# pdh930105/ARCQuant

Hardware: AMD Instinct MI355X
Metric: ARC-NVFP4 GEMM TFLOP/s (M=4096, N=KQ=4096, KE=64) (higher is better)
Workload: dtype f16

## Files before the change

arcquant_amd/csrc/gemm_common.hpp:

```cpp
#pragma once
#include <hip/hip_runtime.h>
#include <stdint.h>

#include "arcq_device.hpp"

#ifdef ARCQ_PLAIN_WEIGHT_LOADS
#define ARCQ_WLOAD(ptr) (*(ptr))
#else
#define ARCQ_WLOAD(ptr) __builtin_nontemporal_load(ptr)
#endif

namespace arcq {

typedef _Float16 f16x2 __attribute__((ext_vector_type(2)));
typedef _Float16 f16x8 __attribute__((ext_vector_type(8)));
typedef float f32x4 __attribute__((ext_vector_type(4)));
typedef float f32x16 __attribute__((ext_vector_type(16)));

union Frag8 {
  f16x8 v;
  f16x2 p[4];
  uint4 u;
};

__device__ __forceinline__ f16x2 sf_pair(uint32_t byte) {
  const uint32_t h = (byte & 0x7fu) << 7;
  const uint32_t w = h | (h << 16);
  f16x2 r;
  __builtin_memcpy(&r, &w, 4);
  return r;
}

__device__ __forceinline__ f16x2 sf_pair_at(uint32_t word, uint32_t off) {
  const uint32_t w = __builtin_amdgcn_ubfe(word, off, 7u) * 0x00800080u;
  f16x2 r;
  __builtin_memcpy(&r, &w, 4);
  return r;
}

__device__ __forceinline__ Frag8 dequant8(uint32_t codes, f16x2 s2) {
  Frag8 f;
#ifdef ARCQ_EXPERIMENT_NO_SCALE_MUL
  f.p[0] = __builtin_amdgcn_cvt_scalef32_pk_f16_fp4(codes, 256.0f, 0);
  f.p[1] = __builtin_amdgcn_cvt_scalef32_pk_f16_fp4(codes, 256.0f, 1);
  f.p[2] = __builtin_amdgcn_cvt_scalef32_pk_f16_fp4(codes, 256.0f, 2);
  f.p[3] = __builtin_amdgcn_cvt_scalef32_pk_f16_fp4(codes, 256.0f, 3);
  (void)s2;
  return f;
#endif
  f.p[0] = __builtin_amdgcn_cvt_scalef32_pk_f16_fp4(codes, 256.0f, 0) * s2;
  f.p[1] = __builtin_amdgcn_cvt_scalef32_pk_f16_fp4(codes, 256.0f, 1) * s2;
  f.p[2] = __builtin_amdgcn_cvt_scalef32_pk_f16_fp4(codes, 256.0f, 2) * s2;
  f.p[3] = __builtin_amdgcn_cvt_scalef32_pk_f16_fp4(codes, 256.0f, 3) * s2;
  return f;
}

__device__ __forceinline__ int64_t sf_atom_offset(int r, int atom, int atoms_k) {
  return ((int64_t)(r >> 7) * atoms_k + atom) * 512 + (r & 31) * 16 + ((r >> 5) & 3) * 4;
}

__device__ __forceinline__ uint32_t pack_bf16x2(float a, float b) { return f32_to_bf16_bits(a) | (f32_to_bf16_bits(b) << 16); }

template <typename Idx, typename P>
__device__ __forceinline__ void store_out4(const P& p, int m, int n, const float (&d)[4]) {
  if (p.out_dtype == ARCQ_OUT_F32) {
    float* o = reinterpret_cast<float*>(p.D) + ((Idx)m * (Idx)p.N + (Idx)n);
    if (n + 3 < p.N && (p.N & 3) == 0) {
      *reinterpret_cast<float4*>(o) = make_float4(d[0], d[1], d[2], d[3]);
    } else {
      for (int r = 0; r < 4; ++r) if (n + r < p.N) o[r] = d[r];
    }
  } else {
    uint16_t* o = reinterpret_cast<uint16_t*>(p.D) + ((Idx)m * (Idx)p.N + (Idx)n);
    if (n + 3 < p.N && (p.N & 3) == 0) {
      *reinterpret_cast<uint2*>(o) = make_uint2(pack_bf16x2(d[0], d[1]), pack_bf16x2(d[2], d[3]));
    } else {
      for (int r = 0; r < 4; ++r) if (n + r < p.N) o[r] = (uint16_t)f32_to_bf16_bits(d[r]);
    }
  }
}

template <typename Idx, typename P>
__device__ __forceinline__ void finish4_pre(const P& p, float alpha, int m, int n, const float (&acc)[4], uint2 bias_bits, uint2 res_bits) {
  const uint32_t bw[2] = {bias_bits.x, bias_bits.y}, rw[2] = {res_bits.x, res_bits.y};
  float d[4];
#pragma unroll
  for (int r = 0; r < 4; ++r) {
    d[r] = alpha * acc[r];
    if (p.bias) {
      const float b = bf16_bits_to_f32((bw[r >> 1] >> (16 * (r & 1))) & 0xffffu);
      d[r] = (p.out_dtype == ARCQ_OUT_F32 ? d[r] : bf16_bits_to_f32(f32_to_bf16_bits(d[r]))) + b;
    }
    if (p.residual) {
      const float res = bf16_bits_to_f32((rw[r >> 1] >> (16 * (r & 1))) & 0xffffu);
      d[r] = (p.out_dtype == ARCQ_OUT_F32 ? d[r] : bf16_bits_to_f32(f32_to_bf16_bits(d[r]))) + res;
    }
  }
  store_out4<Idx>(p, m, n, d);
}

template <typename Idx, typename P>
__device__ __forceinline__ void finish4(const P& p, float alpha, int m, int n, const float (&acc)[4]) {
  if ((p.N & 3) == 0 && (p.bias || p.residual) && ((reinterpret_cast<uintptr_t>(p.bias) | reinterpret_cast<uintptr_t>(p.residual)) & 7) == 0) {
    uint2 b2 = make_uint2(0, 0), r2 = make_uint2(0, 0);
    if (p.bias) b2 = *reinterpret_cast<const uint2*>(p.bias + n);
    if (p.residual) r2 = *reinterpret_cast<const uint2*>(p.residual + ((Idx)m * (Idx)p.N + (Idx)n));
    finish4_pre<Idx>(p, alpha, m, n, acc, b2, r2);
    return;
  }
  float d[4];
#pragma unroll
  for (int r = 0; r < 4; ++r) {
    d[r] = alpha * acc[r];
    if (p.bias && n + r < p.N) {
      const float b = bf16_bits_to_f32(p.bias[n + r]);
      d[r] = (p.out_dtype == ARCQ_OUT_F32 ? d[r] : bf16_bits_to_f32(f32_to_bf16_bits(d[r]))) + b;
    }
    if (p.residual && n + r < p.N) {
      const float res = bf16_bits_to_f32(p.residual[(Idx)m * (Idx)p.N + (Idx)(n + r)]);
      d[r] = (p.out_dtype == ARCQ_OUT_F32 ? d[r] : bf16_bits_to_f32(f32_to_bf16_bits(d[r]))) + res;
    }
  }
  store_out4<Idx>(p, m, n, d);
}

}
```

arcquant_amd/csrc/gemm_rowblock.hip:

```cpp
#include <hip/hip_runtime.h>
#include <stdint.h>
#include <stdlib.h>

#include "arcq_internal.hpp"
#include "gemm_common.hpp"
#include "rowblock_split.hpp"

namespace arcq {

struct RowblockParams {
  const uint8_t* A;
  const uint8_t* SFA;
  const uint8_t* RW;
  const uint8_t* RSF;
  void* D;
  const float* alpha_dev;
  const uint16_t* bias;
  const uint16_t* residual;
  int M, N, K;
  float alpha_host;
  int out_dtype;
  int pairs;
  int row_blocks;
  int slices;
  int a_stride;
  unsigned int* silu_slots;
};

typedef uint32_t rb_u32x4 __attribute__((ext_vector_type(4)));
struct RowblockRegs {
  rb_u32x4 b0, b1;
  uint32_t s;
};

constexpr int kRbWaves = 8, kRbThreads = kRbWaves * 64;

template <int kUnits, bool kSiluAbsmax>
__global__ __launch_bounds__(kRbThreads, 4) void gemm_rowblock_kernel(RowblockParams p) {
  extern __shared__ __attribute__((aligned(16))) unsigned char smem[];
  unsigned char* const a_img = smem;
  float* const red = reinterpret_cast<float*>(smem);

  const int tid = threadIdx.x, lane = tid & 63, wave = tid >> 6;
  const int q = lane >> 4, rl = lane & 15;
  const int bpw = kRbWaves / p.slices;
  const int rb = blockIdx.x * bpw + wave / p.slices;
  const int slice = wave % p.slices;
  const bool active = rb < p.row_blocks;
  int pr_begin, pr_count;
  rowblock_slice_range(p.pairs, p.slices, slice, &pr_begin, &pr_count);
  const int npairs = active ? pr_count : 0;
  const float alpha = p.alpha_host * (p.alpha_dev ? *p.alpha_dev : 1.0f);

  const int upr = p.pairs * 8, real = p.K >> 5;
  const int atoms_k = p.K >> 6;
  const int units = p.M * upr;
  uint4 qv_pre[kUnits];
  uint32_t sf_pre[kUnits];
#pragma unroll
  for (int j = 0; j < kUnits; ++j) {
    const int u = min(tid + j * kRbThreads, units - 1);
    const int m = u / upr, c = min(u - m * upr, real - 1);
    qv_pre[j] = *reinterpret_cast<const uint4*>(p.A + (size_t)m * (p.K >> 1) + c * 16);
    sf_pre[j] = *reinterpret_cast<const uint32_t*>(p.SFA + sf_atom_offset(m, c >> 1, atoms_k));
  }

  const int rbc = active ? rb : 0;
  const int pr_load = rowblock_load_base(pr_begin, npairs);
  const uint8_t* wp = p.RW + ((size_t)rbc * p.pairs + pr_load) * 2048 + lane * 16;
  const uint8_t* sp = p.RSF + ((size_t)rbc * p.pairs + pr_load) * 256 + lane * 4;
  const int last = npairs > 0 ? npairs - 1 : 0;
  int issued = 0;
  auto issue = [&](RowblockRegs& r) __attribute__((always_inline)) {
    const int i = min(issued, last);
    r.b0 = ARCQ_WLOAD(reinterpret_cast<const rb_u32x4*>(wp + (size_t)i * 2048));
    r.b1 = ARCQ_WLOAD(reinterpret_cast<const rb_u32x4*>(wp + (size_t)i * 2048 + 1024));
    r.s = ARCQ_WLOAD(reinterpret_cast<const uint32_t*>(sp + (size_t)i * 256));
    ++issued;
  };
  RowblockRegs r0, r1, r2;
  issue(r0);
  issue(r1);
  issue(r2);

  auto put_unit = [&](int u, uint4 qv, uint32_t sf) __attribute__((always_inline)) {
    const int m = u / upr, c = u - m * upr;
    uint4 f0 = make_uint4(0, 0, 0, 0), f1 = f0, f2 = f0, f3 = f0;
    if (c < real) {
      sf >>= (c & 1) * 16;
      const f16x2 s0 = sf_pair_at(sf, 0), s1 = sf_pair_at(sf, 8);
      f0 = dequant8(qv.x, s0).u; f1 = dequant8(qv.y, s0).u; f2 = dequant8(qv.z, s1).u; f3 = dequant8(qv.w, s1).u;
    }
    uint4* dst = reinterpret_cast<uint4*>(a_img + (size_t)m * p.a_stride + c * 64);
    dst[0] = f0; dst[1] = f1; dst[2] = f2; dst[3] = f3;
  };
#pragma unroll
  for (int j = 0; j < kUnits; ++j) {
    const int u = tid + j * kRbThreads;
    if (u < units) put_unit(u, qv_pre[j], sf_pre[j]);
  }
  for (int u = tid + kUnits * kRbThreads; u < units; u += kRbThreads) {
    const int m = u / upr, c = min(u - m * upr, real - 1);
    put_unit(u, *reinterpret_cast<const uint4*>(p.A + (size_t)m * (p.K >> 1) + c * 16),
             *reinterpret_cast<const uint32_t*>(p.SFA + sf_atom_offset(m, c >> 1, atoms_k)));
  }
  __syncthreads();

  f32x4 acc = {0.f, 0.f, 0.f, 0.f};
  const unsigned char* a_lane = a_img + (size_t)min(rl, p.M - 1) * p.a_stride + (size_t)pr_begin * 512 + q * 64;
  int done = 0;
  auto tile = [&](rb_u32x4 b, uint32_t s16, const unsigned char* ap) __attribute__((always_inline)) {
    Frag8 a0, a1, a2, a3;
    a0.u = *reinterpret_cast<const uint4*>(ap);
    a1.u = *reinterpret_cast<const uint4*>(ap + 16);
    a2.u = *reinterpret_cast<const uint4*>(ap + 32);
    a3.u = *reinterpret_cast<const uint4*>(ap + 48);
    const f16x2 s0 = sf_pair_at(s16, 0), s1 = sf_pair_at(s16, 8);
    const Frag8 b0 = dequant8(b.x, s0), b1 = dequant8(b.y, s0), b2 = dequant8(b.z, s1), b3 = dequant8(b.w, s1);
    acc = __builtin_amdgcn_mfma_f32_16x16x32_f16(b0.v, a0.v, acc, 0, 0, 0);
    acc = __builtin_amdgcn_mfma_f32_16x16x32_f16(b1.v, a1.v, acc, 0, 0, 0);
    acc = __builtin_amdgcn_mfma_f32_16x16x32_f16(b2.v, a2.v, acc, 0, 0, 0);
    acc = __builtin_amdgcn_mfma_f32_16x16x32_f16(b3.v, a3.v, acc, 0, 0, 0);
  };
  auto step = [&](RowblockRegs& r) __attribute__((always_inline)) {
    const unsigned char* ap = a_lane + (size_t)done * 512;
    tile(r.b0, r.s, ap);
    tile(r.b1, r.s >> 16, ap + 256);
    issue(r);
    __builtin_amdgcn_sched_barrier(0);
    ++done;
  };
  typedef uint32_t rb_u32x2 __attribute__((ext_vector_type(2)));
  rb_u32x2 ep_bias = {0, 0}, ep_res = {0, 0};
  const bool ep_pre = !kSiluAbsmax && (p.N & 3) == 0 && (p.bias || p.residual);
  if (ep_pre && slice == 0 && active && rl < p.M && rb * 16 + 4 * q < p.N) {
    const int n0p = rb * 16 + 4 * q;
    if (p.bias) ep_bias = *reinterpret_cast<const rb_u32x2*>(p.bias + n0p);
    if (p.residual) ep_res = *reinterpret_cast<const rb_u32x2*>(p.residual + (size_t)rl * p.N + n0p);
  }
#pragma unroll 1
  while (done + 3 <= npairs) {
    step(r0);
    step(r1);
    step(r2);
  }
  if (done < npairs) step(r0);
  if (done < npairs) step(r1);

  float sum[4] = {acc[0], acc[1], acc[2], acc[3]};
  if (p.slices > 1) {
    __syncthreads();
    *reinterpret_cast<float4*>(red + (wave * 64 + lane) * 4) = make_float4(sum[0], sum[1], sum[2], sum[3]);
    __syncthreads();
    if (slice != 0) return;
    for (int s2 = 1; s2 < p.slices; ++s2) {
      const float4 v = *reinterpret_cast<const float4*>(red + ((wave + s2) * 64 + lane) * 4);
      sum[0] += v.x; sum[1] += v.y; sum[2] += v.z; sum[3] += v.w;
    }
  }
  const int n0 = rb * 16 + 4 * q;
  if (active && rl < p.M && n0 < p.N) {
    if (ep_pre) finish4_pre<uint32_t>(p, alpha, rl, n0, sum, make_uint2(ep_bias.x, ep_bias.y), make_uint2(ep_res.x, ep_res.y));
    else finish4<uint32_t>(p, alpha, rl, n0, sum);
  }
  if constexpr (kSiluAbsmax) {
    uint32_t m = 0;
    if (active && rl < p.M && n0 < p.N) {
      const uint32_t b0 = f32_to_bf16_bits(alpha * sum[0]), b1 = f32_to_bf16_bits(alpha * sum[1]);
      const uint32_t b2 = f32_to_bf16_bits(alpha * sum[2]), b3 = f32_to_bf16_bits(alpha * sum[3]);
      m = max(silu_mul_bf16(b0, b1) & 0x7fffu, silu_mul_bf16(b2, b3) & 0x7fffu);
    }
#pragma unroll
    for (int sh = 32; sh > 0; sh >>= 1) m = max(m, (uint32_t)__shfl_down((int)m, sh, 64));
    if (lane == 0 && active) p.silu_slots[rb] = m;
  }
}

struct RowblockActRegs {
  rb_u32x4 a0, a1;
  uint32_t s0, s1;
};

template <bool kSiluAbsmax>
__global__ __launch_bounds__(kRbThreads, 2) void gemm_rowblock_direct_kernel(RowblockParams p) {
  extern __shared__ __attribute__((aligned(16))) unsigned char smem[];
  float* const red = reinterpret_cast<float*>(smem);

  const int tid = threadIdx.x, lane = tid & 63, wave = tid >> 6;
  const int q = lane >> 4, rl = lane & 15;
  const int bpw = kRbWaves / p.slices;
  const int rb = blockIdx.x * bpw + wave / p.slices;
  const int slice = wave % p.slices;
  const bool active = rb < p.row_blocks;
  int pr_begin, pr_count;
  rowblock_slice_range(p.pairs, p.slices, slice, &pr_begin, &pr_count);
  const int npairs = active ? pr_count : 0;
  const float alpha = p.alpha_host * (p.alpha_dev ? *p.alpha_dev : 1.0f);

  const int rbc = active ? rb : 0;
  const int pr_load = rowblock_load_base(pr_begin, npairs);
  const uint8_t* wp = p.RW + ((size_t)rbc * p.pairs + pr_load) * 2048 + lane * 16;
  const uint8_t* sp = p.RSF + ((size_t)rbc * p.pairs + pr_load) * 256 + lane * 4;
  const int tok = min(rl, p.M - 1);
  const int atoms_k = p.K >> 6, tiles_k = p.K >> 7;
  const uint8_t* arow = p.A + (size_t)tok * (p.K >> 1) + q * 16;
  const uint8_t* srow = p.SFA + sf_atom_offset(tok, 0, atoms_k) + (q & 1) * 2;
  const int last = npairs > 0 ? npairs - 1 : 0;
  int issued = 0;
  auto issue = [&](RowblockRegs& r, RowblockActRegs& x) __attribute__((always_inline)) {
    const int i = min(issued, last);
    const int t0 = 2 * (pr_load + i), t1 = t0 + 1;
    const int halfk = (p.K & 64) ? 1 : 0;
    auto a_off = [&](int t) __attribute__((always_inline)) -> size_t {
      const int tc = min(t, tiles_k - 1 + halfk);
      size_t off = (size_t)tc * 64;
      if (halfk && tc == tiles_k && q >= 2) off -= 32;
      return off;
    };
    auto s_off = [&](int t) __attribute__((always_inline)) -> size_t {
      const int atom = min(2 * t + (q >> 1), atoms_k - 1);
      return (size_t)atom * 512;
    };
    x.a0 = *reinterpret_cast<const rb_u32x4*>(arow + a_off(t0));
    x.a1 = *reinterpret_cast<const rb_u32x4*>(arow + a_off(t1));
    x.s0 = *reinterpret_cast<const uint16_t*>(srow + s_off(t0));
    x.s1 = *reinterpret_cast<const uint16_t*>(srow + s_off(t1));
    r.b0 = ARCQ_WLOAD(reinterpret_cast<const rb_u32x4*>(wp + (size_t)i * 2048));
    r.b1 = ARCQ_WLOAD(reinterpret_cast<const rb_u32x4*>(wp + (size_t)i * 2048 + 1024));
    r.s = ARCQ_WLOAD(reinterpret_cast<const uint32_t*>(sp + (size_t)i * 256));
    ++issued;
// ... 156 lines not shown
```

arcquant_amd/csrc/gemm_stream.hip:

```cpp
#include <type_traits>
#include <hip/hip_runtime.h>
#include <stdint.h>
#include <stdlib.h>

#include "arcq_internal.hpp"
#include "gemm_common.hpp"
#include "quantize_device.hpp"
#include "stream_split.hpp"

namespace arcq {

#ifdef ARCQ_STREAM_STAMPS
static unsigned long long* g_stream_stamps = nullptr;
extern "C" void arcq_debug_set_stream_stamps(void* p) { g_stream_stamps = reinterpret_cast<unsigned long long*>(p); }
#define ARCQ_STAMP(i)                                                                                                   \
  do {                                                                                                                  \
    if (p.stamps) {                                                                                                     \
      __builtin_amdgcn_sched_barrier(0);                                                                                \
      unsigned long long t_;                                                                                            \
      asm volatile("s_memtime %0\n\ts_waitcnt lgkmcnt(0)" : "=s"(t_)::"memory");                                        \
      __builtin_amdgcn_sched_barrier(0);                                                                                \
      if (lane == 0) p.stamps[((size_t)blockIdx.x * kStreamWaves + wave) * 16 + (i)] = t_;                               \
    }                                                                                                                   \
  } while (0)
#define ARCQ_STAMP_RT(i)                                                                                                \
  do {                                                                                                                  \
    if (p.stamps) {                                                                                                     \
      unsigned long long t_;                                                                                            \
      asm volatile("s_memrealtime %0\n\ts_waitcnt lgkmcnt(0)" : "=s"(t_)::"memory");                                    \
      if (lane == 0) p.stamps[((size_t)blockIdx.x * kStreamWaves + wave) * 16 + (i)] = t_;                              \
    }                                                                                                                   \
  } while (0)
#else
#define ARCQ_STAMP(i) do { } while (0)
#define ARCQ_STAMP_RT(i) do { } while (0)
#endif

enum : int { kSrcPacked = 0, kSrcRms = 1, kSrcDyn = 2 };
enum : int { kOutPlain = 0, kOutSiluAbsmax = 1, kOutSiluAct = 2 };

struct StreamParams {
  const uint8_t* RW;
  const uint8_t* RSF;
  const uint8_t* A;
  const uint8_t* SFA;
  const uint16_t* X;
  const uint16_t* Wn;
  const int16_t* idx;
  const uint32_t* in_slots;
  float* scale_out;
  float eps;
  int KQ, KE, n_in_slots;
  void* D;
  const float* alpha_dev;
  const uint16_t* bias;
  const uint16_t* residual;
  uint32_t* out_slots;
  const int16_t* act_scatter;
  int M, N, K;
  float alpha_host;
  int out_dtype;
  int pairs;
  int row_blocks;
  int a_stride;
  int img_bytes;
  int stage;
  int xrow_bytes;
  int slot_off;
  int stage_off, misc_off;
#ifdef ARCQ_STREAM_STAMPS
  unsigned long long* stamps;
#endif
};

typedef uint32_t st_u32x4 __attribute__((ext_vector_type(4)));
typedef uint32_t st_u32x2 __attribute__((ext_vector_type(2)));
struct StreamRegs {
  st_u32x4 b0, b1;
  uint32_t s;
};

constexpr int kStThreads = kStreamWaves * 64;
constexpr int kStSlotBytes = kStreamWaves * 2 * 64 * 16;
constexpr int kStMiscBytes = 1024;

__device__ __forceinline__ void image_put_unit(unsigned char* a_img, const StreamParams& p, int u, int upr, int real, uint4 qv, uint32_t sf) {
  const int m = u / upr, c = u - m * upr;
  uint4 f0 = make_uint4(0, 0, 0, 0), f1 = f0, f2 = f0, f3 = f0;
  if (c < real) {
    sf >>= (c & 1) * 16;
    const f16x2 s0 = sf_pair_at(sf, 0), s1 = sf_pair_at(sf, 8);
    f0 = dequant8(qv.x, s0).u; f1 = dequant8(qv.y, s0).u; f2 = dequant8(qv.z, s1).u; f3 = dequant8(qv.w, s1).u;
  }
  uint4* dst = reinterpret_cast<uint4*>(a_img + (size_t)m * p.a_stride + c * 64);
  dst[0] = f0; dst[1] = f1; dst[2] = f2; dst[3] = f3;
}

__device__ __forceinline__ void image_put_group(unsigned char* a_img, const StreamParams& p, int m, int pos, const GroupQ& g) {
  const f16x2 s2 = sf_pair(g.s8);
  uint4* dst = reinterpret_cast<uint4*>(a_img + (size_t)m * p.a_stride + (size_t)pos * 32);
  dst[0] = dequant8(g.packed.x, s2).u;
  dst[1] = dequant8(g.packed.y, s2).u;
}

constexpr int kTask = 6;

__device__ __forceinline__ uint4 asm_load_b128(const void* ptr) {
  st_u32x4 v;
  asm volatile("global_load_dwordx4 %0, %1, off" : "=v"(v) : "v"(ptr) : "memory");
  return make_uint4(v.x, v.y, v.z, v.w);
}
__device__ __forceinline__ uint32_t asm_load_b32(const void* ptr) {
  uint32_t v;
  asm volatile("global_load_dword %0, %1, off" : "=v"(v) : "v"(ptr) : "memory");
  return v;
}
__device__ __forceinline__ void asm_wait_behind_units(int units) {
  switch (units) {
    case 0: asm volatile("s_waitcnt vmcnt(0)" ::: "memory"); break;
    case 1: asm volatile("s_waitcnt vmcnt(3)" ::: "memory"); break;
    case 2: asm volatile("s_waitcnt vmcnt(6)" ::: "memory"); break;
    case 3: asm volatile("s_waitcnt vmcnt(9)" ::: "memory"); break;
    case 4: asm volatile("s_waitcnt vmcnt(12)" ::: "memory"); break;
    case 5: asm volatile("s_waitcnt vmcnt(15)" ::: "memory"); break;
    default: asm volatile("s_waitcnt vmcnt(18)" ::: "memory"); break;
  }
}
__device__ __forceinline__ void asm_tie(uint4& v) { asm volatile("" : "+v"(v.x), "+v"(v.y), "+v"(v.z), "+v"(v.w)); }
__device__ __forceinline__ void asm_tie(uint32_t& v) { asm volatile("" : "+v"(v)); }

template <int kSrc, int kOut, int kVariant>
__global__ __launch_bounds__(kStThreads) void gemm_stream_kernel(StreamParams p) {
  extern __shared__ __attribute__((aligned(16))) unsigned char smem[];
  unsigned char* const a_img = smem;
  float* const slots = reinterpret_cast<float*>(smem + p.slot_off);
  unsigned char* const xstage = smem + p.stage_off;
  float* const misc = reinterpret_cast<float*>(smem + p.misc_off);
  uint32_t* const misc_u = reinterpret_cast<uint32_t*>(misc);

  const int tid = threadIdx.x, lane = tid & 63;
  const int wave = __builtin_amdgcn_readfirstlane(tid >> 6);
  const int q = lane >> 4, rl = lane & 15;

  int rb0, nrb;
  stream_wg_range(p.row_blocks, (int)gridDim.x, (int)blockIdx.x, &rb0, &nrb);
  const int P = p.pairs;
  const int U = nrb * P;
  int u0, n;
  stream_wave_range(U, wave, &u0, &n);
  const int rbl0 = u0 / P;
  const int pa0 = u0 - rbl0 * P;
  const int len1 = min(n, P - pa0);

  float alpha = p.alpha_host * (p.alpha_dev ? *p.alpha_dev : 1.0f);
  ARCQ_STAMP(0);
  ARCQ_STAMP_RT(10);

  const int G = p.KQ >> 4, Ptail = (p.KQ - p.KE) >> 4, Rg = G - Ptail;
  constexpr int kPre = 2;
  uint4 pre_q[kPre];
  uint32_t pre_s[kPre];
  uint4 pre_wn = make_uint4(0, 0, 0, 0), pre_i0 = make_uint4(0, 0, 0, 0), pre_i1 = make_uint4(0, 0, 0, 0);
  uint32_t pre_slot[4] = {0, 0, 0, 0};
  const int upr = P * 8, real = p.K >> 5, atoms_k = p.K >> 6;
  const int chunks = p.KQ >> 3;
  const int ntask_q = p.M * (G + Rg);
  auto qtask = [&](int t, int& m, int& g) __attribute__((always_inline)) -> bool {
    if (t < p.M * G) { m = t / G; g = t - m * G; return false; }
    const int r = t - p.M * G;
    m = r / Rg; g = Ptail + (r - m * Rg);
    return true;
  };
  float s8[8] = {0.f, 0.f, 0.f, 0.f, 0.f, 0.f, 0.f, 0.f};
  int first_m = 0, first_g = 0;
  bool first_twin = false;
  if constexpr (kSrc == kSrcPacked) {
    const int units = p.M * upr;
#pragma unroll
    for (int j = 0; j < kPre; ++j) {
      const int u = min(tid + j * kStThreads, units - 1);
      const int m = u / upr, c = min(u - m * upr, real - 1);
      pre_q[j] = asm_load_b128(p.A + (size_t)m * (p.K >> 1) + c * 16);
      pre_s[j] = asm_load_b32(p.SFA + sf_atom_offset(m, c >> 1, atoms_k));
    }
  } else {
    const int bdx = chunks >> 1;
    if constexpr (kSrc == kSrcRms) {
      pre_wn = *reinterpret_cast<const uint4*>(p.Wn + (size_t)min(tid, chunks - 1) * 8);
    } else {
      const int vt = min(tid, p.M * bdx - 1), m = vt / bdx, v = vt - m * bdx;
      pre_q[0] = *reinterpret_cast<const uint4*>(p.X + ((size_t)m * chunks + v) * 8);
      pre_q[1] = *reinterpret_cast<const uint4*>(p.X + ((size_t)m * chunks + bdx + v) * 8);
      const uint32_t* sl = p.in_slots ? p.in_slots : reinterpret_cast<const uint32_t*>(p.X);
      const int ns = p.in_slots ? p.n_in_slots : 1;
#pragma unroll
      for (int j = 0; j < 4; ++j) pre_slot[j] = sl[min(tid + j * kStThreads, ns - 1)];
    }
    {
      first_twin = qtask(min(tid, ntask_q - 1), first_m, first_g);
      pre_i0 = *reinterpret_cast<const uint4*>(p.idx + (size_t)first_g * 16);
      pre_i1 = *reinterpret_cast<const uint4*>(p.idx + (size_t)first_g * 16 + 8);
    }
    if constexpr (kSrc == kSrcRms) {
      if (wave < p.M) {
        const uint16_t* xrow = p.X + (size_t)wave * p.KQ;
        uint16_t* row = reinterpret_cast<uint16_t*>(xstage + (size_t)wave * p.xrow_bytes);
        uint4 xa[8], xb[8];
#pragma unroll
        for (int j = 0; j < 8; ++j) {
          if (64 * j < bdx) {
            const int v = min(lane + 64 * j, bdx - 1);
            xa[j] = *reinterpret_cast<const uint4*>(xrow + (size_t)v * 8);
            xb[j] = *reinterpret_cast<const uint4*>(xrow + (size_t)(bdx + v) * 8);
          }
        }
#pragma unroll
        for (int j = 0; j < 8; ++j) {
          const int v = lane + 64 * j;
          if (v < bdx) {
            lds_put_chunk(row, v, xa[j]);
            lds_put_chunk(row, bdx + v, xb[j]);
            const uint32_t w8[8] = {xa[j].x, xa[j].y, xa[j].z, xa[j].w, xb[j].x, xb[j].y, xb[j].z, xb[j].w};
            float acc = 0.0f;
#pragma unroll
            for (int e = 0; e < 8; ++e) {
              const float a = bf16_bits_to_f32(w8[e] & 0xffffu), b = bf16_bits_to_f32(w8[e] >> 16);
              acc = acc + a * a;
              acc = acc + b * b;
            }
            s8[j] = acc;
          }
        }
      }
    }
    __builtin_amdgcn_sched_barrier(0);
    if constexpr (kSrc == kSrcRms) {
      asm_tie(pre_wn);
    } else {
      asm_tie(pre_q[0]); asm_tie(pre_q[1]);
#pragma unroll
      for (int j = 0; j < 4; ++j) asm_tie(pre_slot[j]);
    }
    asm_tie(pre_i0); asm_tie(pre_i1);
  }
  __builtin_amdgcn_sched_barrier(0);

  const uint8_t* const wp = p.RW + ((size_t)rb0 * P + u0) * 2048 + lane * 16;
  const uint8_t* const sp = p.RSF + ((size_t)rb0 * P + u0) * 256 + lane * 4;
  auto load_unit = [&](StreamRegs& r, int i) __attribute__((always_inline)) {
    r.b0 = ARCQ_WLOAD(reinterpret_cast<const st_u32x4*>(wp + (size_t)i * 2048));
    r.b1 = ARCQ_WLOAD(reinterpret_cast<const st_u32x4*>(wp + (size_t)i * 2048 + 1024));
    r.s = ARCQ_WLOAD(reinterpret_cast<const uint32_t*>(sp + (size_t)i * 256));
  };
  st_u32x2 ep_bias0 = {0, 0}, ep_bias1 = {0, 0}, ep_res0 = {0, 0}, ep_res1 = {0, 0};
  const bool ep_pre = (kOut == kOutPlain || kOut == kOutSiluAct) && (p.N & 3) == 0 && (p.bias || p.residual);
  auto prefetch_epilogue = [&]() __attribute__((always_inline)) {
    if (!ep_pre) return;
#pragma unroll
    for (int seg = 0; seg < 2; ++seg) {
      const int seg_n = seg == 0 ? len1 : n - len1;
      if (seg_n <= 0 || (seg == 0 && pa0 != 0)) continue;
      const int n0 = (rb0 + rbl0 + seg) * 16 + 4 * q;
      if (rl < p.M && n0 < p.N) {
        if (p.bias) (seg == 0 ? ep_bias0 : ep_bias1) = *reinterpret_cast<const st_u32x2*>(p.bias + n0);
        if (p.residual) (seg == 0 ? ep_res0 : ep_res1) = *reinterpret_cast<const st_u32x2*>(p.residual + (size_t)rl * p.N + n0);
      }
    }
  };
  const int ntasks = (n + kTask - 1) / kTask;
  int task_left = ntasks, done = 0;
  int c = ntasks > 0 ? (n + ntasks - 1) / ntasks : 0;
  StreamRegs r0 = {}, r1 = {}, r2 = {}, r3 = {}, r4 = {}, r5 = {};
  auto load_task_part = [&](int lo, int hi) __attribute__((always_inline)) {
    if (c > 0 && lo <= 0 && 0 < hi) load_unit(r0, done);
    if (c > 1 && lo <= 1 && 1 < hi) load_unit(r1, done + 1);
    if (c > 2 && lo <= 2 && 2 < hi) load_unit(r2, done + 2);
    if (c > 3 && lo <= 3 && 3 < hi) load_unit(r3, done + 3);
    if (c > 4 && lo <= 4 && 4 < hi) load_unit(r4, done + 4);
    if (c > 5 && lo <= 5 && 5 < hi) load_unit(r5, done + 5);
  };
  auto load_task = [&]() __attribute__((always_inline)) { load_task_part(0, kTask); };
  constexpr int kPart = kSrc == kSrcPacked ? kTask : 2;
  const bool token_wave = kSrc == kSrcRms && wave < p.M;
  if (!token_wave) load_task_part(0, kPart);
  __builtin_amdgcn_sched_barrier(0);
  if constexpr (kSrc == kSrcPacked) {
    asm_wait_behind_units(c);
#pragma unroll
    for (int j = 0; j < kPre; ++j) { asm_tie(pre_q[j]); asm_tie(pre_s[j]); }
    __builtin_amdgcn_sched_barrier(0);
  }
  ARCQ_STAMP(1);
  if (ntasks <= 1) prefetch_epilogue();

  if constexpr (kSrc == kSrcPacked) {
    const int units = p.M * upr;
#pragma unroll
    for (int j = 0; j < kPre; ++j) {
      const int u = tid + j * kStThreads;
      if (u < units) image_put_unit(a_img, p, u, upr, real, pre_q[j], pre_s[j]);
    }
    for (int u = tid + kPre * kStThreads; u < units; u += kStThreads) {
      const int m = u / upr, cc = min(u - m * upr, real - 1);
      image_put_unit(a_img, p, u, upr, real, *reinterpret_cast<const uint4*>(p.A + (size_t)m * (p.K >> 1) + cc * 16),
                     *reinterpret_cast<const uint32_t*>(p.SFA + sf_atom_offset(m, cc >> 1, atoms_k)));
    }
  } else {
    uint32_t amax = 0;
    const int bdx = chunks >> 1;
    if constexpr (kSrc == kSrcRms) {
      if (wave < p.M) {
#pragma unroll
        for (int j = 0; j < 4; ++j) s8[j] = s8[j] + s8[j + 4];
        s8[0] = s8[0] + s8[2];
        s8[1] = s8[1] + s8[3];
        float z = s8[0] + s8[1];
        const float up = __shfl_down(z, 32, 64);
        if (lane < 32) z = z + up;
        float val = lane < 32 ? z : 0.0f;
        val += __shfl_down(val, 16, 64);
        val += dpp_row_shl<8>(val);
        val += dpp_row_shl<4>(val);
        val += dpp_row_shl<2>(val);
        val += dpp_row_shl<1>(val);
        if (lane == 0) {
          const float var = val / (float)p.KQ + p.eps;
          misc[32 + wave] = (float)(1.0 / sqrt((double)var));
        }
      }
      if (tid < chunks) lds_put_chunk(reinterpret_cast<uint16_t*>(xstage + (size_t)p.M * p.xrow_bytes), tid, pre_wn);
      for (int cidx = tid + kStThreads; cidx < chunks; cidx += kStThreads)
        lds_put_chunk(reinterpret_cast<uint16_t*>(xstage + (size_t)p.M * p.xrow_bytes), cidx, *reinterpret_cast<const uint4*>(p.Wn + (size_t)cidx * 8));
      ARCQ_STAMP(8);
      __syncthreads();
    } else {
      const int vthreads = p.M * bdx;
      const bool need = p.stage || !p.in_slots;
      if (need) {
        for (int t = tid; t < vthreads; t += kStThreads) {
          const int m = t / bdx, v = t - m * bdx;
          uint4 d0 = pre_q[0], d1 = pre_q[1];
          if (t != tid) {
            d0 = *reinterpret_cast<const uint4*>(p.X + ((size_t)m * chunks + v) * 8);
            d1 = *reinterpret_cast<const uint4*>(p.X + ((size_t)m * chunks + bdx + v) * 8);
          }
          if (p.stage) {
            uint16_t* row = reinterpret_cast<uint16_t*>(xstage + (size_t)m * p.xrow_bytes);
            lds_put_chunk(row, v, d0);
            lds_put_chunk(row, bdx + v, d1);
          }
          amax = absmax_bits_chunk(d1, absmax_bits_chunk(d0, amax));
        }
      }
    }
// ... 9 lines not shown
      __syncthreads();
      uint32_t mbits = 0;
#pragma unroll
      for (int w = 0; w < kStreamWaves; ++w) mbits = max(mbits, misc_u[w]);
      dyn_scale = bf16_bits_to_f32(mbits) * (1.0f / (448.0f * 6.0f));
      if (blockIdx.x == 0 && tid == 0 && p.scale_out) p.scale_out[0] = dyn_scale;
      alpha *= dyn_scale;
      dyn_scale = round_to_bf16(dyn_scale);
    }
    const DynDiv dyn_div(dyn_scale, kSrc == kSrcDyn);
    load_task_part(token_wave ? 0 : kPart, 2 * kPart);
    __builtin_amdgcn_sched_barrier(0);
    ARCQ_STAMP(9);
    const uint16_t* wn_lds = reinterpret_cast<const uint16_t*>(xstage + (size_t)p.M * p.xrow_bytes);
    const st_u32x4 pi0 = {pre_i0.x, pre_i0.y, pre_i0.z, pre_i0.w}, pi1 = {pre_i1.x, pre_i1.y, pre_i1.z, pre_i1.w};
    auto run_groups = [&](auto stage_tag, auto fast_tag) __attribute__((always_inline)) {
    constexpr bool kStage = decltype(stage_tag)::value, kFast = decltype(fast_tag)::value;
    for (int t = tid; t < ntask_q; t += kStThreads) {
      int m = first_m, g = first_g;
      bool twin = first_twin;
      st_u32x4 i0 = pi0, i1 = pi1;
      if (t != tid) {
        twin = qtask(t, m, g);
        i0 = *reinterpret_cast<const st_u32x4*>(p.idx + (size_t)g * 16);
        i1 = *reinterpret_cast<const st_u32x4*>(p.idx + (size_t)g * 16 + 8);
      }
      const uint32_t iw[8] = {i0.x, i0.y, i0.z, i0.w, i1.x, i1.y, i1.z, i1.w};
      const uint16_t* xrow_lds = reinterpret_cast<const uint16_t*>(xstage + (size_t)m * p.xrow_bytes);
      const uint16_t* xrow_g = p.X + (size_t)m * p.KQ;
      const float rstd = kSrc == kSrcRms ? misc[32 + m] : 1.0f;
      float v[16];
#pragma unroll
      for (int j = 0; j < 8; ++j) {
        const uint32_t ia = iw[j] & 0xffffu, ib = iw[j] >> 16;
        const uint32_t pw = lds_pad_pair(iw[j]), pa = pw & 0xffffu, pb = pw >> 16;
        float a, b;
        if (kStage) {
          a = bf16_bits_to_f32(xrow_lds[pa]);
          b = bf16_bits_to_f32(xrow_lds[pb]);
        } else {
          a = bf16_bits_to_f32(xrow_g[ia]);
          b = bf16_bits_to_f32(xrow_g[ib]);
        }
        if (kSrc == kSrcDyn) {
          a = round_to_bf16(dyn_div.template div<kFast>(a));
          b = round_to_bf16(dyn_div.template div<kFast>(b));
        }
        if (kSrc == kSrcRms) {
          a = round_to_bf16(a * bf16_bits_to_f32(wn_lds[pa]) * rstd);
          b = round_to_bf16(b * bf16_bits_to_f32(wn_lds[pb]) * rstd);
        }
        v[2 * j] = a;
        v[2 * j + 1] = b;
      }
      int pos;
      if (kVariant == ARCQ_VARIANT_G16) {
        pos = g + (g > Ptail ? g - Ptail : 0);
      } else {
        const int g1 = g & ~1;
        pos = g1 + (g1 > Ptail ? g1 - Ptail : 0) + (g & 1);
      }
      if (!twin) {
        image_put_group(a_img, p, m, pos, quantize_group<false, kVariant>(v));
      } else {
        quantize_group<true, kVariant>(v);
        image_put_group(a_img, p, m, pos + (kVariant == ARCQ_VARIANT_G16 ? 1 : 2), quantize_group<false, kVariant>(v));
      }
    }
    };
    if constexpr (kSrc == kSrcRms) {
      run_groups(std::true_type{}, std::true_type{});
    } else if (p.stage) {
      if (dyn_div.fast) run_groups(std::true_type{}, std::true_type{});
      else run_groups(std::true_type{}, std::false_type{});
    } else {
      if (dyn_div.fast) run_groups(std::false_type{}, std::true_type{});
      else run_groups(std::false_type{}, std::false_type{});
    }
    load_task_part(2 * kPart, kTask);
    __builtin_amdgcn_sched_barrier(0);
    const int pad_groups = P * 16 - (p.K >> 4);
    for (int t = tid; t < p.M * pad_groups; t += kStThreads) {
      const int m = t / pad_groups, g = (p.K >> 4) + (t - m * pad_groups);
      uint4* dst = reinterpret_cast<uint4*>(a_img + (size_t)m * p.a_stride + (size_t)g * 32);
      dst[0] = make_uint4(0, 0, 0, 0);
      dst[1] = make_uint4(0, 0, 0, 0);
    }
  }
  ARCQ_STAMP(2);
  __syncthreads();
  ARCQ_STAMP(3);

  f32x4 acc = {0.f, 0.f, 0.f, 0.f}, acc1 = {0.f, 0.f, 0.f, 0.f};
  const unsigned char* const a_tok = a_img + (size_t)min(rl, p.M - 1) * p.a_stride + q * 64;
  int pr = pa0;
  auto tile = [&](st_u32x4 b, uint32_t s16, const unsigned char* ap) __attribute__((always_inline)) {
    Frag8 a0, a1, a2, a3;
    a0.u = *reinterpret_cast<const uint4*>(ap);
    a1.u = *reinterpret_cast<const uint4*>(ap + 16);
    a2.u = *reinterpret_cast<const uint4*>(ap + 32);
    a3.u = *reinterpret_cast<const uint4*>(ap + 48);
    const f16x2 s0 = sf_pair_at(s16, 0), s1 = sf_pair_at(s16, 8);
    const Frag8 b0 = dequant8(b.x, s0), b1 = dequant8(b.y, s0), b2 = dequant8(b.z, s1), b3 = dequant8(b.w, s1);
    acc = __builtin_amdgcn_mfma_f32_16x16x32_f16(b0.v, a0.v, acc, 0, 0, 0);
    acc = __builtin_amdgcn_mfma_f32_16x16x32_f16(b1.v, a1.v, acc, 0, 0, 0);
    acc = __builtin_amdgcn_mfma_f32_16x16x32_f16(b2.v, a2.v, acc, 0, 0, 0);
    acc = __builtin_amdgcn_mfma_f32_16x16x32_f16(b3.v, a3.v, acc, 0, 0, 0);
  };
  auto step = [&](const StreamRegs& r) __attribute__((always_inline)) {
    const unsigned char* ap = a_tok + (size_t)pr * 512;
    tile(r.b0, r.s, ap);
    tile(r.b1, r.s >> 16, ap + 256);
    ++done;
    ++pr;
    if (done == len1) {
      acc1 = acc;
      acc = f32x4{0.f, 0.f, 0.f, 0.f};
      pr = 0;
    }
  };
#pragma unroll 1
  while (task_left > 0) {
    const int cc = c;
    if (cc > 0) step(r0);
    if (cc > 1) step(r1);
    if (cc > 2) step(r2);
    if (cc > 3) step(r3);
    if (cc > 4) step(r4);
    if (cc > 5) step(r5);
    if (--task_left > 0) {
      c = (n - done + task_left - 1) / task_left;
      load_task();
      if (task_left == 1) prefetch_epilogue();
    }
  }
  ARCQ_STAMP(4);

  if (p.slot_off == 0) __syncthreads();
  {
    float* mine = slots + ((wave * 2) * 64 + lane) * 4;
    *reinterpret_cast<float4*>(mine) = make_float4(acc1[0], acc1[1], acc1[2], acc1[3]);
    *reinterpret_cast<float4*>(mine + 64 * 4) = make_float4(acc[0], acc[1], acc[2], acc[3]);
  }
  __syncthreads();
  ARCQ_STAMP(5);
#pragma unroll 1
  for (int seg = 0; seg < 2; ++seg) {
    const int seg_n = seg == 0 ? len1 : n - len1;
    if (seg_n <= 0 || (seg == 0 && pa0 != 0)) continue;
    const int rbl = seg == 0 ? rbl0 : rbl0 + 1;
    float4 sum = *reinterpret_cast<const float4*>(slots + ((wave * 2 + seg) * 64 + lane) * 4);
    const int rb_end = (rbl + 1) * P;
    for (int w2 = wave + 1; w2 < kStreamWaves; ++w2) {
      const int s2 = stream_wave_start(U, w2), e2 = stream_wave_start(U, w2 + 1);
      if (s2 >= rb_end) break;
      if (e2 > s2) {
        const float4 v = *reinterpret_cast<const float4*>(slots + ((w2 * 2) * 64 + lane) * 4);
        sum.x += v.x; sum.y += v.y; sum.z += v.z; sum.w += v.w;
      }
    }
    const int rb = rb0 + rbl;
    const int n0 = rb * 16 + 4 * q;
    const bool live = rl < p.M && n0 < p.N;
    const float sv[4] = {sum.x, sum.y, sum.z, sum.w};
    if constexpr (kOut == kOutSiluAct) {
      uint32_t mx = 0;
      if (live) {
        uint32_t y[4];
        const st_u32x2 eb = seg == 0 ? ep_bias0 : ep_bias1;
        const uint32_t bw[2] = {eb.x, eb.y};
#pragma unroll
        for (int e = 0; e < 4; ++e) {
          y[e] = f32_to_bf16_bits(alpha * sv[e]);
          if (p.bias) y[e] = f32_to_bf16_bits(bf16_bits_to_f32(y[e]) + bf16_bits_to_f32((bw[e >> 1] >> (16 * (e & 1))) & 0xffffu));
        }
        const uint32_t a0 = silu_mul_bf16(y[0], y[1]);
        const uint32_t a1 = silu_mul_bf16(y[2], y[3]);
        uint16_t* arow = reinterpret_cast<uint16_t*>(p.D) + (size_t)rl * (p.N >> 1);
        if (p.act_scatter) {
          const uint32_t jj = *reinterpret_cast<const uint32_t*>(p.act_scatter + (n0 >> 1));
          arow[jj & 0xffffu] = (uint16_t)a0;
          arow[jj >> 16] = (uint16_t)a1;
        } else {
          *reinterpret_cast<uint32_t*>(arow + (n0 >> 1)) = a0 | (a1 << 16);
        }
        mx = max(a0 & 0x7fffu, a1 & 0x7fffu);
      }
      mx = wave_max_u32(mx);
      if (lane == 0) p.out_slots[rb] = mx;
    } else {
      if (live) {
        if (ep_pre) {
          const st_u32x2 eb = seg == 0 ? ep_bias0 : ep_bias1, er = seg == 0 ? ep_res0 : ep_res1;
          finish4_pre<uint32_t>(p, alpha, rl, n0, sv, make_uint2(eb.x, eb.y), make_uint2(er.x, er.y));
        }
        else finish4<uint32_t>(p, alpha, rl, n0, sv);
      }
      if constexpr (kOut == kOutSiluAbsmax) {
        uint32_t mx = 0;
        if (live) {
          const uint32_t b0 = f32_to_bf16_bits(alpha * sv[0]), b1 = f32_to_bf16_bits(alpha * sv[1]);
          const uint32_t b2 = f32_to_bf16_bits(alpha * sv[2]), b3 = f32_to_bf16_bits(alpha * sv[3]);
          mx = max(silu_mul_bf16(b0, b1) & 0x7fffu, silu_mul_bf16(b2, b3) & 0x7fffu);
        }
        mx = wave_max_u32(mx);
        if (lane == 0) p.out_slots[rb] = mx;
      }
    }
  }
  ARCQ_STAMP(6);
  ARCQ_STAMP_RT(11);
}

static int64_t stream_pairs(int64_t K) { return (K + 255) / 256; }
// ... 108 lines not shown
```

Measured before the change: 1419.

## Use buffer loads, swizzle A image in LDS, and simplify task scheduling

```diff
diff --git a/arcquant_amd/csrc/gemm_common.hpp b/arcquant_amd/csrc/gemm_common.hpp
--- a/arcquant_amd/csrc/gemm_common.hpp
+++ b/arcquant_amd/csrc/gemm_common.hpp
@@ -8,6 +8,11 @@
 #define ARCQ_WLOAD(ptr) (*(ptr))
 #else
 #define ARCQ_WLOAD(ptr) __builtin_nontemporal_load(ptr)
+#endif
+#ifdef ARCQ_PLAIN_WEIGHT_LOADS
+#define ARCQ_WLOAD_AUX 0
+#else
+#define ARCQ_WLOAD_AUX 2
 #endif
 
 namespace arcq {
@@ -58,6 +63,8 @@
 __device__ __forceinline__ int64_t sf_atom_offset(int r, int atom, int atoms_k) {
   return ((int64_t)(r >> 7) * atoms_k + atom) * 512 + (r & 31) * 16 + ((r >> 5) & 3) * 4;
 }
+
+__device__ __forceinline__ int image_unit_flip(int token) { return ((token + 4) >> 3) & 1; }
 
 __device__ __forceinline__ uint32_t pack_bf16x2(float a, float b) { return f32_to_bf16_bits(a) | (f32_to_bf16_bits(b) << 16); }
 
diff --git a/arcquant_amd/csrc/gemm_rowblock.hip b/arcquant_amd/csrc/gemm_rowblock.hip
--- a/arcquant_amd/csrc/gemm_rowblock.hip
+++ b/arcquant_amd/csrc/gemm_rowblock.hip
@@ -35,13 +35,15 @@
 
 constexpr int kRbWaves = 8, kRbThreads = kRbWaves * 64;
 
+
 template <int kUnits, bool kSiluAbsmax>
 __global__ __launch_bounds__(kRbThreads, 4) void gemm_rowblock_kernel(RowblockParams p) {
   extern __shared__ __attribute__((aligned(16))) unsigned char smem[];
   unsigned char* const a_img = smem;
   float* const red = reinterpret_cast<float*>(smem);
 
-  const int tid = threadIdx.x, lane = tid & 63, wave = tid >> 6;
+  const int tid = threadIdx.x, lane = tid & 63;
+  const int wave = __builtin_amdgcn_readfirstlane(tid >> 6);
   const int q = lane >> 4, rl = lane & 15;
   const int bpw = kRbWaves / p.slices;
   const int rb = blockIdx.x * bpw + wave / p.slices;
@@ -65,23 +67,35 @@
     sf_pre[j] = *reinterpret_cast<const uint32_t*>(p.SFA + sf_atom_offset(m, c >> 1, atoms_k));
   }
 
+  typedef uint32_t rb_u32x2 __attribute__((ext_vector_type(2)));
+  rb_u32x2 ep_bias = {0, 0}, ep_res = {0, 0};
+  const bool ep_pre = !kSiluAbsmax && (p.N & 3) == 0 && (p.bias || p.residual);
+  if (ep_pre && slice == 0 && active && rl < p.M && rb * 16 + 4 * q < p.N) {
+    const int n0p = rb * 16 + 4 * q;
+    if (p.bias) ep_bias = *reinterpret_cast<const rb_u32x2*>(p.bias + n0p);
+    if (p.residual) ep_res = *reinterpret_cast<const rb_u32x2*>(p.residual + (size_t)rl * p.N + n0p);
+  }
+
   const int rbc = active ? rb : 0;
   const int pr_load = rowblock_load_base(pr_begin, npairs);
-  const uint8_t* wp = p.RW + ((size_t)rbc * p.pairs + pr_load) * 2048 + lane * 16;
-  const uint8_t* sp = p.RSF + ((size_t)rbc * p.pairs + pr_load) * 256 + lane * 4;
-  const int last = npairs > 0 ? npairs - 1 : 0;
-  int issued = 0;
+  const auto rs_w = __builtin_amdgcn_make_buffer_rsrc(const_cast<uint8_t*>(p.RW + ((size_t)rbc * p.pairs + pr_load) * 2048), 0, npairs * 2048, 0x00020000);
+  const auto rs_s = __builtin_amdgcn_make_buffer_rsrc(const_cast<uint8_t*>(p.RSF + ((size_t)rbc * p.pairs + pr_load) * 256), 0, npairs * 256, 0x00020000);
+  const uint32_t wlane = (uint32_t)lane * 16u, slane = (uint32_t)lane * 4u;
+  int wcur = 0, scur = 0;
   auto issue = [&](RowblockRegs& r) __attribute__((always_inline)) {
-    const int i = min(issued, last);
-    r.b0 = ARCQ_WLOAD(reinterpret_cast<const rb_u32x4*>(wp + (size_t)i * 2048));
-    r.b1 = ARCQ_WLOAD(reinterpret_cast<const rb_u32x4*>(wp + (size_t)i * 2048 + 1024));
-    r.s = ARCQ_WLOAD(reinterpret_cast<const uint32_t*>(sp + (size_t)i * 256));
-    ++issued;
+    r.b0 = __builtin_amdgcn_raw_buffer_load_b128(rs_w, wlane, wcur, ARCQ_WLOAD_AUX);
+    r.b1 = __builtin_amdgcn_raw_buffer_load_b128(rs_w, wlane + 1024u, wcur, ARCQ_WLOAD_AUX);
+    r.s = __builtin_amdgcn_raw_buffer_load_b32(rs_s, slane, scur, ARCQ_WLOAD_AUX);
+    wcur += 2048;
+    scur += 256;
   };
   RowblockRegs r0, r1, r2;
   issue(r0);
+  __builtin_amdgcn_sched_barrier(0);
   issue(r1);
+  __builtin_amdgcn_sched_barrier(0);
   issue(r2);
+  __builtin_amdgcn_sched_barrier(0);
 
   auto put_unit = [&](int u, uint4 qv, uint32_t sf) __attribute__((always_inline)) {
     const int m = u / upr, c = u - m * upr;
@@ -91,7 +105,7 @@
       const f16x2 s0 = sf_pair_at(sf, 0), s1 = sf_pair_at(sf, 8);
       f0 = dequant8(qv.x, s0).u; f1 = dequant8(qv.y, s0).u; f2 = dequant8(qv.z, s1).u; f3 = dequant8(qv.w, s1).u;
     }
-    uint4* dst = reinterpret_cast<uint4*>(a_img + (size_t)m * p.a_stride + c * 64);
+    uint4* dst = reinterpret_cast<uint4*>(a_img + (size_t)m * p.a_stride + (c ^ image_unit_flip(m)) * 64);
     dst[0] = f0; dst[1] = f1; dst[2] = f2; dst[3] = f3;
   };
 #pragma unroll
@@ -107,8 +121,7 @@
   __syncthreads();
 
   f32x4 acc = {0.f, 0.f, 0.f, 0.f};
-  const unsigned char* a_lane = a_img + (size_t)min(rl, p.M - 1) * p.a_stride + (size_t)pr_begin * 512 + q * 64;
-  int done = 0;
+  const unsigned char* a_lane = a_img + (size_t)min(rl, p.M - 1) * p.a_stride + (size_t)pr_begin * 512 + (q ^ image_unit_flip(rl)) * 64;
   auto tile = [&](rb_u32x4 b, uint32_t s16, const unsigned char* ap) __attribute__((always_inline)) {
     Frag8 a0, a1, a2, a3;
     a0.u = *reinterpret_cast<const uint4*>(ap);
@@ -122,30 +135,37 @@
     acc = __builtin_amdgcn_mfma_f32_16x16x32_f16(b2.v, a2.v, acc, 0, 0, 0);
     acc = __builtin_amdgcn_mfma_f32_16x16x32_f16(b3.v, a3.v, acc, 0, 0, 0);
   };
-  auto step = [&](RowblockRegs& r) __attribute__((always_inline)) {
-    const unsigned char* ap = a_lane + (size_t)done * 512;
+  auto consume = [&](const RowblockRegs& r, const unsigned char* ap) __attribute__((always_inline)) {
     tile(r.b0, r.s, ap);
     tile(r.b1, r.s >> 16, ap + 256);
+  };
+  auto refill = [&](RowblockRegs& r) __attribute__((always_inline)) {
     issue(r);
     __builtin_amdgcn_sched_barrier(0);
-    ++done;
-  };
-  typedef uint32_t rb_u32x2 __attribute__((ext_vector_type(2)));
-  rb_u32x2 ep_bias = {0, 0}, ep_res = {0, 0};
-  const bool ep_pre = !kSiluAbsmax && (p.N & 3) == 0 && (p.bias || p.residual);
-  if (ep_pre && slice == 0 && active && rl < p.M && rb * 16 + 4 * q < p.N) {
-    const int n0p = rb * 16 + 4 * q;
-    if (p.bias) ep_bias = *reinterpret_cast<const rb_u32x2*>(p.bias + n0p);
-    if (p.residual) ep_res = *reinterpret_cast<const rb_u32x2*>(p.residual + (size_t)rl * p.N + n0p);
-  }
+  };
+  int left = npairs;
 #pragma unroll 1
-  while (done + 3 <= npairs) {
-    step(r0);
-    step(r1);
-    step(r2);
-  }
-  if (done < npairs) step(r0);
-  if (done < npairs) step(r1);
+  while (left >= 6) {
+    consume(r0, a_lane);
+    refill(r0);
+    consume(r1, a_lane + 512);
+    refill(r1);
+    consume(r2, a_lane + 1024);
+    refill(r2);
+    a_lane += 1536;
+    left -= 3;
+  }
+  if (left > 0) {
+    consume(r0, a_lane);
+    if (left > 3) refill(r0);
+  }
+  if (left > 1) {
+    consume(r1, a_lane + 512);
+    if (left > 4) refill(r1);
+  }
+  if (left > 2) consume(r2, a_lane + 1024);
+  if (left > 3) consume(r0, a_lane + 1536);
+  if (left > 4) consume(r1, a_lane + 2048);
 
   float sum[4] = {acc[0], acc[1], acc[2], acc[3]};
   if (p.slices > 1) {
diff --git a/arcquant_amd/csrc/gemm_stream.hip b/arcquant_amd/csrc/gemm_stream.hip
--- a/arcquant_amd/csrc/gemm_stream.hip
+++ b/arcquant_amd/csrc/gemm_stream.hip
@@ -75,6 +75,8 @@
 
 typedef uint32_t st_u32x4 __attribute__((ext_vector_type(4)));
 typedef uint32_t st_u32x2 __attribute__((ext_vector_type(2)));
+typedef __attribute__((address_space(1))) st_u32x4 st_global_u32x4;
+typedef __attribute__((address_space(1))) uint32_t st_global_u32;
 struct StreamRegs {
   st_u32x4 b0, b1;
   uint32_t s;
@@ -92,13 +94,13 @@
     const f16x2 s0 = sf_pair_at(sf, 0), s1 = sf_pair_at(sf, 8);
     f0 = dequant8(qv.x, s0).u; f1 = dequant8(qv.y, s0).u; f2 = dequant8(qv.z, s1).u; f3 = dequant8(qv.w, s1).u;
   }
-  uint4* dst = reinterpret_cast<uint4*>(a_img + (size_t)m * p.a_stride + c * 64);
+  uint4* dst = reinterpret_cast<uint4*>(a_img + (size_t)m * p.a_stride + (c ^ image_unit_flip(m)) * 64);
   dst[0] = f0; dst[1] = f1; dst[2] = f2; dst[3] = f3;
 }
 
 __device__ __forceinline__ void image_put_group(unsigned char* a_img, const StreamParams& p, int m, int pos, const GroupQ& g) {
   const f16x2 s2 = sf_pair(g.s8);
-  uint4* dst = reinterpret_cast<uint4*>(a_img + (size_t)m * p.a_stride + (size_t)pos * 32);
+  uint4* dst = reinterpret_cast<uint4*>(a_img + (size_t)m * p.a_stride + (size_t)(pos ^ (image_unit_flip(m) << 1)) * 32);
   dst[0] = dequant8(g.packed.x, s2).u;
   dst[1] = dequant8(g.packed.y, s2).u;
 }
@@ -245,12 +247,16 @@
   }
   __builtin_amdgcn_sched_barrier(0);
 
-  const uint8_t* const wp = p.RW + ((size_t)rb0 * P + u0) * 2048 + lane * 16;
-  const uint8_t* const sp = p.RSF + ((size_t)rb0 * P + u0) * 256 + lane * 4;
+  const uint8_t* const wp = p.RW + ((size_t)rb0 * P + u0) * 2048;
+  const uint8_t* const sp = p.RSF + ((size_t)rb0 * P + u0) * 256;
+  uint32_t wlane = (uint32_t)lane * 16u, slane = (uint32_t)lane * 4u;
+  asm("" : "+v"(wlane), "+v"(slane));
   auto load_unit = [&](StreamRegs& r, int i) __attribute__((always_inline)) {
-    r.b0 = ARCQ_WLOAD(reinterpret_cast<const st_u32x4*>(wp + (size_t)i * 2048));
-    r.b1 = ARCQ_WLOAD(reinterpret_cast<const st_u32x4*>(wp + (size_t)i * 2048 + 1024));
-    r.s = ARCQ_WLOAD(reinterpret_cast<const uint32_t*>(sp + (size_t)i * 256));
+    uint64_t wu = reinterpret_cast<uint64_t>(wp + (size_t)i * 2048), su = reinterpret_cast<uint64_t>(sp + (size_t)i * 256);
+    asm("" : "+s"(wu), "+s"(su), "+v"(wlane), "+v"(slane));
+    r.b0 = ARCQ_WLOAD(reinterpret_cast<const st_global_u32x4*>(wu + wlane));
+    r.b1 = ARCQ_WLOAD(reinterpret_cast<const st_global_u32x4*>(wu + 1024 + wlane));
+    r.s = ARCQ_WLOAD(reinterpret_cast<const st_global_u32*>(su + slane));
   };
   st_u32x2 ep_bias0 = {0, 0}, ep_bias1 = {0, 0}, ep_res0 = {0, 0}, ep_res1 = {0, 0};
   const bool ep_pre = (kOut == kOutPlain || kOut == kOutSiluAct) && (p.N & 3) == 0 && (p.bias || p.residual);
@@ -269,7 +275,8 @@
   };
   const int ntasks = (n + kTask - 1) / kTask;
   int task_left = ntasks, done = 0;
-  int c = ntasks > 0 ? (n + ntasks - 1) / ntasks : 0;
+  const int task_base = ntasks > 0 ? n / ntasks : 0, task_big = n - task_base * ntasks;
+  int c = task_base + (task_big > 0 ? 1 : 0);
   StreamRegs r0 = {}, r1 = {}, r2 = {}, r3 = {}, r4 = {}, r5 = {};
   auto load_task_part = [&](int lo, int hi) __attribute__((always_inline)) {
     if (c > 0 && lo <= 0 && 0 < hi) load_unit(r0, done);
@@ -445,7 +452,7 @@
     const int pad_groups = P * 16 - (p.K >> 4);
     for (int t = tid; t < p.M * pad_groups; t += kStThreads) {
       const int m = t / pad_groups, g = (p.K >> 4) + (t - m * pad_groups);
-      uint4* dst = reinterpret_cast<uint4*>(a_img + (size_t)m * p.a_stride + (size_t)g * 32);
+      uint4* dst = reinterpret_cast<uint4*>(a_img + (size_t)m * p.a_stride + (size_t)(g ^ (image_unit_flip(m) << 1)) * 32);
       dst[0] = make_uint4(0, 0, 0, 0);
       dst[1] = make_uint4(0, 0, 0, 0);
     }
@@ -455,7 +462,7 @@
   ARCQ_STAMP(3);
 
   f32x4 acc = {0.f, 0.f, 0.f, 0.f}, acc1 = {0.f, 0.f, 0.f, 0.f};
-  const unsigned char* const a_tok = a_img + (size_t)min(rl, p.M - 1) * p.a_stride + q * 64;
+  const unsigned char* const a_tok = a_img + (size_t)min(rl, p.M - 1) * p.a_stride + (q ^ image_unit_flip(rl)) * 64;
   int pr = pa0;
   auto tile = [&](st_u32x4 b, uint32_t s16, const unsigned char* ap) __attribute__((always_inline)) {
     Frag8 a0, a1, a2, a3;
@@ -476,9 +483,11 @@
     tile(r.b1, r.s >> 16, ap + 256);
     ++done;
     ++pr;
-    if (done == len1) {
+    if (__builtin_expect(done == len1, 0)) {
       acc1 = acc;
+      asm volatile("" : "+v"(acc1));
       acc = f32x4{0.f, 0.f, 0.f, 0.f};
+      asm volatile("" : "+v"(acc));
       pr = 0;
     }
   };
@@ -492,7 +501,7 @@
     if (cc > 4) step(r4);
     if (cc > 5) step(r5);
     if (--task_left > 0) {
-      c = (n - done + task_left - 1) / task_left;
+      c = task_base + (ntasks - task_left < task_big ? 1 : 0);
       load_task();
       if (task_left == 1) prefetch_epilogue();
     }
```

New measurement: 1419, median of 3. No clear change (-0.0%).
